# PhucNguyenAH/tacotron2_subword

Hardware: AMD Instinct MI355X
Metric: mel_frames_per_sec_train (higher is better)
Workload: dtype bf16; 1 GPU; BERT_Tacotron2 default hparams (SMA), full training iteration fwd+loss+bwd+clip+Adam, B=64/GPU, 100 phones, 60 sub-word tokens, 400 frames, 80-mel; global_batch=64, frames_per_item=400, parallelism=dp1, torch_ops=loss reductions, cat/transpose copies, persistent_chains=True, recurrent_steps_bf16=True

## Files before the change

### include/t2amd.h

```cpp
#ifndef T2AMD_H
#define T2AMD_H
#include <stddef.h>
#include <stdint.h>

#ifdef __cplusplus
extern "C" {
#endif

#define T2_ATTN_SMA 0
#define T2_ATTN_LSA 1
#define T2_ATTN_DCA 4
#define T2_ATTN_GMM 3
#define T2_ATTN_FWD2 2

enum {
    T2_SITE_PRENET1 = 1, T2_SITE_PRENET2 = 2, T2_SITE_PRENET1_SUB = 3, T2_SITE_PRENET2_SUB = 4,
    T2_SITE_ATT_H = 5, T2_SITE_ATT_C = 6, T2_SITE_ATT_H_SUB = 7, T2_SITE_ATT_C_SUB = 8,
    T2_SITE_DEC_H = 9, T2_SITE_DEC_C = 10, T2_SITE_NOISE = 11, T2_SITE_NOISE_SUB = 12,
    T2_SITE_ENC0 = 16,
    T2_SITE_ENCSUB0 = 20,
    T2_SITE_POSTNET0 = 24
};

const char* t2_last_error(void);
#define T2_ABI_VERSION 4
int t2_version(void);
int t2_chain_status(uint32_t* out_host );
int t2_chain_status_clear(void);
int t2_debug_report_abort(uint32_t code, void* stream);
int t2_debug_occupy(int workgroups, int milliseconds, void* stream);
int t2_chain_claimed(void);
int t2_set_precision(int mode);
int t2_get_precision(void);
int t2_gemm_counts(uint64_t* out_host , int reset);
int t2_set_gemm_split_min_mflop(int mflop);
int t2_set_split_steps(int on);
int t2_get_split_steps(void);
int t2_step_counts(uint64_t* out_host , int reset);
int t2_set_overlap(int on);
int t2_set_chain(int on);
int t2_get_chain(void);
int t2_set_chain_bwd(int on);
int t2_set_gemm_staging(int on);
int t2_set_gemm_fold(int on);
int t2_set_bn_fuse(int on);
int t2_get_bn_fuse(void);
int t2_bn_fuse_counts(uint64_t* out_host , int reset);
int t2_side_join(void* stream);

typedef struct t2_dims {
    int n_mel;
    int prenet_dim;
    int enc_dim;
    int att_rnn_dim;
    int dec_rnn_dim;
    int att_dim;
    int loc_filters;
    int loc_kernel;
    int attention_kind;
    float p_att_dropout, p_dec_dropout, p_prenet_dropout;
    int n_streams;
    float score_mask_value, score_mask_value_sub;
    int score_mask_given;
} t2_dims;

typedef struct t2_attention_weights {
    const float* wq;
    const float* wm;
    const float* v;
    const float* loc_conv;
    const float* loc_dense;
    const float* mlp_b1;
    const float* mlp_w2;
    const float* mlp_b2;
    const float* dca_T;
    const float* dca_bT;
    const float* dca_P;
} t2_attention_weights;
typedef struct t2_lstm_weights { const float *w_ih, *w_hh, *b_ih, *b_hh; } t2_lstm_weights;
typedef struct t2_decoder_weights {
    const float *prenet_w1, *prenet_w2;
// ... 323 lines not shown
```

### tacotron2_subword_amd/_lib.py

```python
from __future__ import annotations

import ctypes as C
import os

import torch

_HERE = os.path.dirname(os.path.abspath(__file__))
LIB_PATH = os.environ.get("T2AMD_LIB") or os.path.join(_HERE, "libt2amd.so")

ATTN_SMA, ATTN_LSA, ATTN_FWD2, ATTN_GMM, ATTN_DCA = 0, 1, 2, 3, 4

SITE = dict(PRENET1=1, PRENET2=2, PRENET1_SUB=3, PRENET2_SUB=4, ATT_H=5, ATT_C=6, ATT_H_SUB=7, ATT_C_SUB=8,
            DEC_H=9, DEC_C=10, NOISE=11, NOISE_SUB=12, ENC0=16, ENCSUB0=20, POSTNET0=24)

_fp = C.POINTER(C.c_float)
_ip = C.POINTER(C.c_int32)


class Dims(C.Structure):
    _fields_ = [("n_mel", C.c_int), ("prenet_dim", C.c_int), ("enc_dim", C.c_int), ("att_rnn_dim", C.c_int),
                ("dec_rnn_dim", C.c_int), ("att_dim", C.c_int), ("loc_filters", C.c_int), ("loc_kernel", C.c_int),
                ("attention_kind", C.c_int), ("p_att_dropout", C.c_float), ("p_dec_dropout", C.c_float),
                ("p_prenet_dropout", C.c_float), ("n_streams", C.c_int),
                ("score_mask_value", C.c_float), ("score_mask_value_sub", C.c_float), ("score_mask_given", C.c_int)]
# ... 178 lines not shown


class VocoderConvArgs(C.Structure):
    _fields_ = [("B", C.c_int), ("Cin", C.c_int), ("Cout", C.c_int), ("L", C.c_int), ("k", C.c_int), ("d", C.c_int), ("u", C.c_int),
                ("x", C.c_void_p), ("w", C.c_void_p), ("bias", C.c_void_p), ("residual", C.c_void_p),
                ("y", C.c_void_p), ("packed_ws", C.c_void_p),
                ("slope", C.c_float), ("accumulate", C.c_int), ("scale", C.c_float)]


VOCODER_TIME_TILE = 128


class StftPlanInfo(C.Structure):
    _fields_ = [("bins", C.c_int), ("overlap", C.c_int), ("frame_tile", C.c_int), ("bin_tile", C.c_int), ("out_len", C.c_long),
                ("fwd_floats", C.c_size_t), ("inv_floats", C.c_size_t), ("wsq_floats", C.c_size_t), ("packed_bytes", C.c_size_t)]


class StftAnalysisArgs(C.Structure):
    _fields_ = [("B", C.c_int), ("N", C.c_int), ("hop", C.c_int), ("n", C.c_long), ("x", C.c_void_p), ("packed", C.c_void_p),
                ("re", C.c_void_p), ("im", C.c_void_p), ("mag", C.c_void_p), ("phase", C.c_void_p)]


class StftSynthesisArgs(C.Structure):
    _fields_ = [("B", C.c_int), ("N", C.c_int), ("hop", C.c_int), ("nf", C.c_int), ("mode", C.c_int), ("windowed", C.c_int),
                ("a", C.c_void_p), ("b", C.c_void_p), ("bias", C.c_void_p), ("strength", C.c_float),
                ("packed", C.c_void_p), ("y", C.c_void_p)]


STFT_FRAME_TILE = 32
STFT_POLAR, STFT_DENOISE = 0, 1

ABI_VERSION = 4

EXPORTS = ["t2_last_error", "t2_version", "t2_chain_status", "t2_chain_status_clear", "t2_debug_report_abort", "t2_debug_occupy", "t2_chain_claimed", "t2_set_precision", "t2_get_precision", "t2_gemm_counts", "t2_set_gemm_split_min_mflop", "t2_set_split_steps", "t2_get_split_steps", "t2_step_counts", "t2_set_overlap", "t2_set_chain", "t2_get_chain", "t2_set_chain_bwd", "t2_set_gemm_staging", "t2_set_gemm_fold", "t2_set_bn_fuse", "t2_get_bn_fuse", "t2_bn_fuse_counts", "t2_side_join", "t2_decoder_layout_query", "t2_decoder_forward", "t2_decoder_infer",
           "t2_decoder_bwd_layout_query", "t2_decoder_backward", "t2_prof_enable", "t2_prof_collect", "t2_adam_chunks", "t2_adam_step", "t2_adam_norm",
           "t2_conv_bn_forward", "t2_conv_bn_backward", "t2_embedding_forward", "t2_embedding_backward",
           "t2_lstm_seq_forward", "t2_lstm_seq_backward", "t2_lstm_seq_chain_ws_floats", "t2_gemm_ex", "t2_prof_gemm", "t2_gemm_plan", "t2_conv_handoff_plan", "t2_colsum", "t2_mask_btc",
           "t2_finalize_bct", "t2_mask_bt", "t2_gemm", "t2_rng_keep_mask", "t2_rng_normal",
           "t2_softdtw_plan", "t2_softdtw_dist", "t2_softdtw_forward", "t2_softdtw_backward", "t2_softdtw_dist_backward",
           "t2_hifigan_plan", "t2_hifigan_pack", "t2_hifigan_forward", "t2_vocoder_packed_floats", "t2_vocoder_conv1d", "t2_vocoder_conv_transpose1d",
           "t2_stft_plan", "t2_stft_pack", "t2_stft_analysis", "t2_stft_synthesis"]

_lib = None


def lib() -> C.CDLL:
    global _lib
    if _lib is None:
        if not os.path.exists(LIB_PATH):
            raise RuntimeError(f"{LIB_PATH} is missing: the HIP extension must be built (see __graft_entry__.build); "
                               "there is no CPU fallback for the product path")
        L = C.CDLL(LIB_PATH)
        L.t2_last_error.restype = C.c_char_p
        if L.t2_version() != ABI_VERSION:
            raise RuntimeError(f"{LIB_PATH} speaks ABI version {L.t2_version()}, this binding {ABI_VERSION}: rebuild the library "
                               "(the argument structs differ in size between versions)")
        L.t2_chain_status.argtypes = [C.POINTER(C.c_uint32)]
        L.t2_debug_report_abort.argtypes = [C.c_uint32, C.c_void_p]
        L.t2_debug_occupy.argtypes = [C.c_int, C.c_int, C.c_void_p]
        L.t2_gemm.argtypes = [C.c_void_p, C.c_void_p, C.c_void_p, C.c_int, C.c_int, C.c_int, C.c_long, C.c_long, C.c_long,
                              C.c_long, C.c_long, C.c_void_p, C.c_int, C.c_float, C.c_float, C.c_void_p, C.c_size_t,
                              C.c_int, C.c_void_p]
        L.t2_rng_keep_mask.argtypes = [C.c_uint64, C.c_uint32, C.c_uint32, C.c_float, C.c_void_p, C.c_void_p]
        L.t2_rng_normal.argtypes = [C.c_uint64, C.c_uint32, C.c_uint32, C.c_void_p, C.c_void_p]
        L.t2_decoder_layout_query.argtypes = [C.POINTER(Dims), C.c_int, C.c_int, C.c_int, C.c_int, C.POINTER(DecoderLayout)]
        L.t2_decoder_forward.argtypes = [C.POINTER(Dims), C.POINTER(DecoderWeights), C.POINTER(DecoderFwdArgs), C.c_void_p]
        L.t2_decoder_infer.argtypes = [C.POINTER(Dims), C.POINTER(DecoderWeights), C.POINTER(DecoderInferArgs), C.c_void_p]
        L.t2_decoder_bwd_layout_query.argtypes = [C.POINTER(Dims), C.c_int, C.c_int, C.c_int, C.c_int, C.POINTER(DecoderBwdLayout)]
        L.t2_decoder_backward.argtypes = [C.POINTER(Dims), C.POINTER(DecoderWeights), C.POINTER(DecoderGrads),
                                          C.POINTER(DecoderBwdArgs), C.c_void_p]
        L.t2_conv_bn_forward.argtypes = [C.POINTER(ConvBnArgs), C.c_void_p]
        L.t2_conv_bn_backward.argtypes = [C.POINTER(ConvBnBwdArgs), C.c_void_p]
        L.t2_embedding_forward.argtypes = [C.c_void_p, C.c_void_p, C.c_void_p, C.c_int, C.c_int, C.c_void_p]
        L.t2_embedding_backward.argtypes = [C.c_void_p, C.c_void_p, C.c_void_p, C.c_int, C.c_int, C.c_int, C.c_void_p]
        L.t2_lstm_seq_forward.argtypes = [C.POINTER(LstmSeqArgs), C.c_void_p]
        L.t2_lstm_seq_backward.argtypes = [C.POINTER(LstmSeqBwdArgs), C.c_void_p]
        L.t2_lstm_seq_chain_ws_floats.argtypes, L.t2_lstm_seq_chain_ws_floats.restype = [C.c_int, C.c_int, C.c_int, C.c_int], C.c_size_t
        L.t2_gemm_ex.argtypes = [C.POINTER(GemmArgs), C.c_void_p]
        L.t2_prof_gemm.argtypes = [C.POINTER(GemmArgs), C.c_int, C.POINTER(C.c_float), C.POINTER(C.c_float), C.c_void_p]
        L.t2_gemm_plan.argtypes = [C.POINTER(GemmArgs), C.POINTER(GemmPlanOpts), C.POINTER(GemmPlanInfo)]
        L.t2_conv_handoff_plan.argtypes = [C.POINTER(GemmArgs), C.POINTER(GemmPlanOpts), C.POINTER(C.c_int), C.POINTER(GemmPlanInfo)]
        L.t2_colsum.argtypes = [C.c_void_p, C.c_long, C.c_int, C.c_int, C.c_void_p, C.c_void_p, C.c_void_p]
        L.t2_mask_btc.argtypes = [C.c_void_p, C.c_int, C.c_int, C.c_int, C.c_void_p, C.c_float, C.c_void_p]
        L.t2_prof_enable.argtypes = [C.c_int]
        L.t2_gemm_counts.argtypes = [C.POINTER(C.c_uint64), C.c_int]
        L.t2_set_split_steps.argtypes = [C.c_int]
        L.t2_step_counts.argtypes = [C.POINTER(C.c_uint64), C.c_int]
        L.t2_bn_fuse_counts.argtypes = [C.POINTER(C.c_uint64), C.c_int]
        L.t2_set_gemm_split_min_mflop.argtypes = [C.c_int]
        L.t2_prof_collect.argtypes = [C.c_int, C.POINTER(C.c_double), C.POINTER(C.c_int)]
        L.t2_finalize_bct.argtypes = [C.c_void_p, C.c_void_p, C.c_int, C.c_int, C.c_int, C.c_void_p, C.c_float, C.c_void_p]
        L.t2_mask_bt.argtypes = [C.c_void_p, C.c_int, C.c_int, C.c_void_p, C.c_float, C.c_void_p]
        L.t2_softdtw_plan.argtypes = [C.c_int, C.c_int, C.c_int, C.c_float, C.c_int, C.POINTER(SoftDtwPlanInfo)]
        L.t2_softdtw_dist.argtypes = [C.POINTER(SoftDtwDistArgs), C.c_void_p]
        L.t2_softdtw_forward.argtypes = [C.POINTER(SoftDtwFwdArgs), C.c_void_p]
        L.t2_softdtw_backward.argtypes = [C.POINTER(SoftDtwBwdArgs), C.c_void_p]
        L.t2_softdtw_dist_backward.argtypes = [C.POINTER(SoftDtwDistBwdArgs), C.c_void_p]
        L.t2_hifigan_plan.argtypes = [C.POINTER(HifiganConfig), C.c_int, C.c_int, C.POINTER(HifiganPlanInfo)]
        L.t2_hifigan_pack.argtypes = [C.POINTER(HifiganConfig), C.POINTER(C.c_void_p), C.POINTER(C.c_void_p), C.c_int, C.c_void_p, C.c_void_p]
        L.t2_hifigan_forward.argtypes = [C.POINTER(HifiganConfig), C.POINTER(HifiganFwdArgs), C.c_void_p]
        L.t2_vocoder_packed_floats.argtypes, L.t2_vocoder_packed_floats.restype = [C.c_int, C.c_int, C.c_int, C.c_int], C.c_size_t
        L.t2_vocoder_conv1d.argtypes = [C.POINTER(VocoderConvArgs), C.c_void_p]
        L.t2_vocoder_conv_transpose1d.argtypes = [C.POINTER(VocoderConvArgs), C.c_void_p]
        L.t2_stft_plan.argtypes = [C.c_int, C.c_int, C.c_int, C.POINTER(StftPlanInfo)]
        L.t2_stft_pack.argtypes = [C.c_int, C.c_int, C.c_void_p, C.c_void_p, C.c_void_p, C.c_void_p, C.c_void_p]
        L.t2_stft_analysis.argtypes = [C.POINTER(StftAnalysisArgs), C.c_void_p]
        L.t2_stft_synthesis.argtypes = [C.POINTER(StftSynthesisArgs), C.c_void_p]
        _lib = L
    return _lib


def check(rc: int) -> None:
    if rc != 0:
        raise RuntimeError(f"t2amd call failed ({rc}): {lib().t2_last_error().decode()}")


def ptr(t: torch.Tensor | None) -> int | None:
    if t is None:
        return None
    if not t.is_cuda:
        raise RuntimeError("t2amd: tensors must live on the GPU (no CPU fallback in the product path)")
# ... 204 lines not shown
    check(lib().t2_step_counts(out, int(bool(reset))))
    return tuple(int(v) for v in out)


def gemm_plan(args: GemmArgs, **opts) -> dict:
    o, info = GemmPlanOpts(**opts), GemmPlanInfo()
    check(lib().t2_gemm_plan(C.byref(args), C.byref(o), C.byref(info)))
    return dict(kernel=info.kernel, name=info.name.decode(), split=bool(info.split), splitk=info.splitk, kchunks=info.kchunks,
                a_src=info.a_src, b_src=info.b_src, stage_bytes_a=info.stage_bytes_a, stage_bytes_b=info.stage_bytes_b)


def conv_handoff_plan(args: GemmArgs, **opts) -> dict:
    o, info, taken = GemmPlanOpts(**opts), GemmPlanInfo(), C.c_int(0)
    check(lib().t2_conv_handoff_plan(C.byref(args), C.byref(o), C.byref(taken), C.byref(info)))
    return dict(taken=bool(taken.value), kernel=info.kernel, name=info.name.decode(), split=bool(info.split), splitk=info.splitk,
                kchunks=info.kchunks, a_src=info.a_src, b_src=info.b_src, stage_bytes_a=info.stage_bytes_a, stage_bytes_b=info.stage_bytes_b)


def set_gemm_fold(on: bool) -> None:
    check(lib().t2_set_gemm_fold(1 if on else 0))


def set_bn_fuse(on: bool) -> None:
    check(lib().t2_set_bn_fuse(1 if on else 0))


def get_bn_fuse() -> bool:
    return bool(lib().t2_get_bn_fuse())


def bn_fuse_counts(reset: bool = False):
    out = (C.c_uint64 * 3)()
    check(lib().t2_bn_fuse_counts(out, int(bool(reset))))
    return tuple(int(v) for v in out)


def set_gemm_split_min_mflop(mflop: int = -1) -> None:
    check(lib().t2_set_gemm_split_min_mflop(int(mflop)))


def softdtw_plan(B: int, N: int, M: int, gamma: float = 1.0, need_grad: bool = False) -> SoftDtwPlanInfo:
    info = SoftDtwPlanInfo()
    check(lib().t2_softdtw_plan(B, N, M, gamma, int(bool(need_grad)), C.byref(info)))
    return info


def hifigan_config(h) -> HifiganConfig:
    g = (lambda k: h[k]) if isinstance(h, dict) else (lambda k: getattr(h, k))
    rates, ukernels = list(g("upsample_rates")), list(g("upsample_kernel_sizes"))
    rkernels, rdil = list(g("resblock_kernel_sizes")), [list(d) for d in g("resblock_dilation_sizes")]
    kind = str(g("resblock"))
    if not kind.lstrip("-").isdigit():
        raise RuntimeError(f"hifigan: resblock \"{kind}\" is not \"1\" or \"2\"")
    if len(rates) != len(ukernels) or len(rkernels) != len(rdil):
        raise RuntimeError("hifigan: upsample_rates / upsample_kernel_sizes and resblock_kernel_sizes / resblock_dilation_sizes must pair up")
    if len(rates) > 6 or len(rkernels) > 6:
        raise RuntimeError(f"hifigan: {len(rates)} upsampling stages / {len(rkernels)} resblock kernels, at most 6 each")
    nd = len(rdil[0]) if rdil else 0
    if any(len(d) != nd for d in rdil) or nd > 3:
        raise RuntimeError(f"hifigan: resblock_dilation_sizes={rdil} must hold equally many (at most 3) dilations per kernel")
    c = HifiganConfig()
    c.resblock, c.n_mel, c.upsample_initial_channel = int(kind), 80, int(g("upsample_initial_channel"))
    c.num_upsamples, c.num_kernels, c.num_dilations = len(rates), len(rkernels), nd
    for i, (u, k) in enumerate(zip(rates, ukernels)):
        c.upsample_rates[i], c.upsample_kernel_sizes[i] = int(u), int(k)
    for j, (k, ds) in enumerate(zip(rkernels, rdil)):
# ... 17 lines not shown
```

### tacotron2_subword_amd/csrc/c_api.hip

```cpp
#include <fcntl.h>
#include <stdarg.h>
#include <stdio.h>
#include <sys/file.h>
#include <unistd.h>
#include <stdlib.h>
#include <string.h>

#include "../../include/t2amd.h"
#include "kernels.h"
#include "driver.h"

static thread_local char g_err[512] = "";

void t2_set_error(const char* fmt, ...) {
    va_list ap;
    va_start(ap, fmt);
    vsnprintf(g_err, sizeof(g_err), fmt, ap);
    va_end(ap);
}

#include <algorithm>
#include <mutex>
#include <vector>

using namespace t2;

namespace t2 {
struct Prof {
    bool on = false;
    std::vector<hipEvent_t> ev;
    std::vector<int> kind;
    size_t used = 0;
};
static Prof g_prof;

ProfScope::ProfScope(int kind, hipStream_t st) : s(st), on(g_prof.on && g_prof.used + 2 <= g_prof.ev.size()) {
    if (on) { g_prof.kind[g_prof.used / 2] = kind; (void)hipEventRecord(g_prof.ev[g_prof.used], s); }
}
ProfScope::~ProfScope() {
    if (on) { (void)hipEventRecord(g_prof.ev[g_prof.used + 1], s); g_prof.used += 2; }
}

static Side g_side[16];
int g_overlap = 1;
int g_chain = getenv("T2_CHAIN") ? atoi(getenv("T2_CHAIN")) : 1;
int g_chain_bwd = getenv("T2_CHAIN_BWD") ? atoi(getenv("T2_CHAIN_BWD")) : 1;
uint64_t g_step_counts[6] = {0, 0, 0, 0, 0, 0};
int counted(int rc, int base, int family) { if (rc == 0) ++g_step_counts[base + family]; return rc; }
int g_split_steps = getenv("T2_SPLIT_STEPS") ? atoi(getenv("T2_SPLIT_STEPS")) != 0 : 0;
int side_get(Side** out) {
    int dev = 0;
    T2_CHECK_HIP(hipGetDevice(&dev));
    Side& sd = g_side[dev & 15];
    if (!sd.s) {
        int least = 0, greatest = 0;
        T2_CHECK_HIP(hipDeviceGetStreamPriorityRange(&least, &greatest));
        T2_CHECK_HIP(hipStreamCreateWithPriority(&sd.s, hipStreamNonBlocking, least));
    }
    *out = &sd;
    return 0;
}
static int side_event(Side& sd, size_t i, hipEvent_t* out) {
    while (sd.ev.size() <= i) {
        hipEvent_t e;
        T2_CHECK_HIP(hipEventCreateWithFlags(&e, hipEventDisableTiming));
        sd.ev.push_back(e);
    }
    *out = sd.ev[i];
    return 0;
}
int stream_edge(Side& sd, size_t i, hipStream_t from, hipStream_t to) {
    hipEvent_t e;
    T2_TRY_RC(side_event(sd, i, &e));
    T2_CHECK_HIP(hipEventRecord(e, from));
    T2_CHECK_HIP(hipStreamWaitEvent(to, e, 0));
    return 0;
}

static StopPoll g_poll[16];
int stop_poll_get(StopPoll** out) {
    int dev = 0;
// ... 102 lines not shown
    T2_LAUNCH_CHECK();
    return 0;
}
int t2_set_precision(int mode) {
    T2_REQUIRE(mode >= 0 && mode <= 2, "t2_set_precision: mode must be 0 (fp32), 1 (bf16 operands) or 2 (split-bf16 large GEMMs), not %d", mode);
    set_precision(mode);
    return 0;
}
int t2_get_precision(void) { return get_precision(); }
int t2_set_gemm_split_min_mflop(int mflop) { set_gemm_split_min_mflop(mflop); return 0; }
int t2_gemm_counts(uint64_t* out_host, int reset) {
    T2_REQUIRE(out_host, "null argument");
    gemm_counts(out_host, reset);
    return 0;
}
int t2_set_split_steps(int on) { g_split_steps = on != 0; return 0; }
int t2_get_split_steps(void) { return g_split_steps; }
int t2_step_counts(uint64_t* out_host, int reset) {
    T2_REQUIRE(out_host, "null argument");
    for (int i = 0; i < 6; ++i) { out_host[i] = g_step_counts[i]; if (reset) g_step_counts[i] = 0; }
    return 0;
}
int t2_set_overlap(int on) { g_overlap = on != 0; return 0; }
int t2_set_chain(int on) { g_chain = on != 0; return 0; }
int t2_get_chain(void) { return g_chain; }
int t2_set_chain_bwd(int on) { g_chain_bwd = on != 0; return 0; }
int t2_set_gemm_staging(int on) { set_gemm_staging(on); return 0; }
int t2_set_gemm_fold(int on) { set_gemm_fold(on); return 0; }
int t2_set_bn_fuse(int on) { set_bn_fuse(on); return 0; }
int t2_get_bn_fuse(void) { return get_bn_fuse(); }
int t2_bn_fuse_counts(uint64_t* out_host, int reset) {
    T2_REQUIRE(out_host, "null argument");
    bn_fuse_counts(out_host, reset);
    return 0;
}
int t2_side_join(void* stream) {
    Side* side = nullptr;
    T2_TRY(side_get(&side));
    hipEvent_t e;
    T2_TRY(side_event(*side, 0, &e));
    T2_CHECK_HIP(hipEventRecord(e, side->s));
    T2_CHECK_HIP(hipStreamWaitEvent((hipStream_t)stream, e, 0));
    return 0;
}

int t2_conv_bn_forward(const t2_conv_bn_args* a, void* stream) {
    T2_REQUIRE(a, "null argument");
    const size_t nw = (size_t)a->Cout * a->Cin * a->K;
    T2_REQUIRE(a->ws_floats >= nw + 128 * (size_t)a->Cout, "t2_conv_bn_forward: workspace too small");
    ConvBnFwd f{};
    f.x = a->x; f.B = a->B; f.T = a->T; f.Cin = a->Cin; f.Cout = a->Cout; f.K = a->K;
    f.w = a->w; f.bias = a->bias; f.gamma = a->gamma; f.beta = a->beta; f.run_mean = a->run_mean; f.run_var = a->run_var;
    f.training = a->training; f.eps = a->eps; f.act = a->act; f.drop_p = a->drop_p; f.seed = a->seed; f.site = a->site;
    f.residual = a->residual; f.z = a->z; f.mean = a->mean; f.invstd = a->invstd; f.var = a->var; f.y = a->y;
    f.wperm = a->ws; f.scratch = a->ws + align4(nw);
    const size_t used = align4(nw) + 128 * (size_t)a->Cout;
    if (a->ws_floats > used) { f.gemm_ws = a->ws + used; f.gemm_ws_bytes = (a->ws_floats - used) * sizeof(float); }
    f.handoff = a->handoff; f.x16 = static_cast<const __bf16*>(a->x16); f.y16 = static_cast<__bf16*>(a->y16);
    return conv_bn_fwd(f, (hipStream_t)stream);
}

int t2_conv_bn_backward(const t2_conv_bn_bwd_args* a, void* stream) {
    T2_REQUIRE(a, "null argument");
    const size_t nw = align4((size_t)a->Cout * a->Cin * a->K), ndz = align4((size_t)a->B * a->T * a->Cout), nsc = 128 * (size_t)a->Cout;
    T2_REQUIRE(a->ws_floats >= nw + ndz + nsc, "t2_conv_bn_backward: workspace too small");
    ConvBnBwd f{};
// ... 358 lines not shown
```

### tacotron2_subword_amd/csrc/decoder.hip

```cpp
#include <stdlib.h>
#include <string.h>

#include <algorithm>
#include <mutex>
#include <unordered_map>
#include <vector>

#include "../../include/t2amd.h"
#include "kernels.h"
#include "driver.h"

using namespace t2;

__global__ __launch_bounds__(256) void poison_if_aborted_kernel(const unsigned* __restrict__ status, int nwords, float* __restrict__ a, size_t na,
                                                                float* __restrict__ b, size_t nb) {
    unsigned any = 0;
    for (int i = 0; i < nwords; ++i) any |= status[i];
    if (!any) return;
    const float qnan = __builtin_nanf("");
    for (size_t i = (size_t)blockIdx.x * 256 + threadIdx.x; i < na; i += (size_t)gridDim.x * 256) a[i] = qnan;
    for (size_t i = (size_t)blockIdx.x * 256 + threadIdx.x; i < nb; i += (size_t)gridDim.x * 256) b[i] = qnan;
}

namespace {
// ... 499 lines not shown
    L->dp2 = take(BT * z.P); L->dp2s = take(BT * z.P); L->dp1 = take(BT * z.P);
    L->dmel_t = take(BT * z.M); L->dgate_t = take(BT);
    L->dg16a = take((size_t)2 * z.B * 4 * z.Ha / 2 + 4); L->dg16d = take((size_t)z.B * 4 * z.Hd / 2 + 4);
    L->colsum_ws = take((size_t)64 * 4 * (z.Ha > z.Hd ? z.Ha : z.Hd));
    L->gemm_ws_floats = (size_t)192 << 20;
    if (get_precision() == 2) {
        const size_t h4 = (size_t)4 * std::max(z.Ha, z.Hd), need = 6 * BT * (h4 + z.WD) + ((size_t)256 << 20);
        L->gemm_ws_floats = std::max(L->gemm_ws_floats, align4(need / sizeof(float)));
    }
    L->gemm_ws = take(L->gemm_ws_floats);
    L->chain_floats = chain_bwd_ws_floats(lsa ? CHAIN_LSA : CHAIN_SMA, z.NS, z.B, z.Ha, z.E, z.A, d.loc_filters, d.loc_kernel, z.Hd);
    L->chain = take(L->chain_floats);
    L->total_floats = off;
}

struct BwdStreamRef {
    const t2_lstm_grads* lg; const t2_attention_grads* ag; float *prenet_w1, *prenet_w2;
    const float* d_align; float* d_memory;
    size_t dg, dctx, dq, dv, dpm, carry, carryc, dlconv, dldense, dc, dp2;
};
void bwd_stream_refs(const t2_decoder_grads& g, const t2_decoder_bwd_args& a, const t2_decoder_bwd_layout& BL, BwdStreamRef* st) {
    for (int s = 0; s < 2; ++s) {
        BwdStreamRef& b = st[s];
        b.lg = s ? &g.att_sub : &g.att; b.ag = s ? &g.attn_sub : &g.attn;
        b.prenet_w1 = s ? g.prenet_sub_w1 : g.prenet_w1; b.prenet_w2 = s ? g.prenet_sub_w2 : g.prenet_w2;
        b.d_align = s ? a.d_align_sub : a.d_align; b.d_memory = s ? a.d_memory_sub : a.d_memory;
        b.dg = s ? BL.dgas : BL.dga; b.dctx = s ? BL.dctxs : BL.dctx; b.dq = s ? BL.dqs : BL.dq; b.dv = s ? BL.dvs : BL.dv;
        b.dpm = s ? BL.dpms : BL.dpm; b.carry = s ? BL.carrys : BL.carry; b.carryc = s ? BL.carrycs : BL.carryc;
        b.dlconv = s ? BL.dlconvs : BL.dlconv; b.dldense = s ? BL.dldenses : BL.dldense;
        b.dc = s ? BL.dcas : BL.dca; b.dp2 = s ? BL.dp2s : BL.dp2;
    }
}

struct Bwd {
    const t2_dims& d; const t2_decoder_weights& w; const t2_decoder_grads& g; const t2_decoder_bwd_args& a;
    Sizes z; t2_decoder_layout L; t2_decoder_bwd_layout BL; hipStream_t s;
    const float* W(size_t off) const { return a.ws + off; }
    float* S(size_t off) const { return a.bws + off; }
    long R(int t) const { return (long)t * z.B; }
    bool use16 = false;
    bool split = false;
    hipStream_t sd = nullptr;
    const __bf16* W16(size_t off) const { return reinterpret_cast<const __bf16*>(a.ws + off); }
    __bf16* S16(size_t off) const { return reinterpret_cast<__bf16*>(a.bws + off); }
    float* gemm_ws() const { return a.bws + BL.gemm_ws; }
    size_t gemm_ws_bytes() const { return BL.gemm_ws_floats * sizeof(float); }
    StreamRef st[2]{}; BwdStreamRef bst[2]{};
    ChainBwdDesc cab{}, cbb{}; bool chain_a = false, chain_b = false;
    Side* side = nullptr; bool overlap = false; size_t ne = 0;
};

GemmDesc matmul_nn(const float* X, long ldx, const float* W, long ldw, float* Y, long ldy, int M, int N, int K) {
    return product(X, ldx, 1, W, 1, ldw, Y, ldy, M, N, K);
}
GemmDesc matmul_tn(const Bwd& c, const float* G, long ldg, const float* X, long ldx, float* Y, long ldy, int M, int N, int K) {
    GemmDesc g = product(G, 1, ldg, X, 1, ldx, Y, ldy, M, N, K);
    g.ws = c.gemm_ws(); g.ws_bytes = c.gemm_ws_bytes();
    return g;
}

struct Dg16 {
    bool on; __bf16* p; long H4; float* rest; size_t rest_bytes;
    GemmDesc operand(GemmDesc m, long row0, int kmajor) const {
        if (on) { m.A16 = p + row0 * H4; m.lda16 = H4; m.a16_kmajor = kmajor; m.ws = rest; m.ws_bytes = rest_bytes; }
        return m;
    }
    GemmDesc wgrad(GemmDesc m, long row0) const { return operand(m, row0, 1); }
    GemmDesc igrad(GemmDesc m, long row0) const { return operand(m, row0, 0); }
};
size_t dg16_bytes(const Sizes& z, int H4) { return ((size_t)H4 * z.B * z.T * sizeof(__bf16) + 255) & ~(size_t)255; }
Dg16 dg16_carve(const Bwd& c, bool on, size_t off, int H4) {
    unsigned char* const at = reinterpret_cast<unsigned char*>(c.gemm_ws()) + off;
    const size_t bytes = dg16_bytes(c.z, H4);
    return Dg16{on, reinterpret_cast<__bf16*>(at), H4, reinterpret_cast<float*>(at + bytes), c.gemm_ws_bytes() - off - bytes};
}

int dec_bwd_step(const Bwd& c, int t) {
    const Sizes& z = c.z;
    const int ks = lstm_bwd_ksplit(4 * z.Hd);
    LstmBwdPointDesc p{};
    p.nstreams = 1; p.B = z.B; p.H = z.Hd; p.seed = c.a.seed; p.first = t == z.T - 1;
    p.drop_p = c.a.training ? c.d.p_dec_dropout : 0.f;
    LstmBwdStream& st = p.st[0];
    st.dh1 = c.S(c.BL.ddout) + c.R(t) * z.WO; st.lddh1 = z.WO;
    st.part = c.S(c.BL.partd); st.nparts = ks; st.part_stride = (long)z.B * z.Hd; st.ldpart = z.Hd; st.part_col = 0;
    st.gates = c.W(c.L.gd) + c.R(t) * 4 * z.Hd; st.ldgates = 4 * z.Hd;
    st.c_new = c.W(c.L.cnd) + c.R(t) * z.Hd; st.ldc_new = z.Hd;
    if (t > 0) { st.c_prev = c.W(c.L.cd) + c.R(t - 1) * z.Hd; st.ldc_prev = z.Hd; }
    st.dc_state = c.S(c.BL.dcd);
    st.dg = c.S(c.BL.dgd) + c.R(t) * 4 * z.Hd; st.lddg = 4 * z.Hd;
    st.site_h = T2_SITE_DEC_H; st.site_c = T2_SITE_DEC_C;
    st.idx_base = (uint32_t)(c.R(t) * z.Hd); st.idx_bstride = (uint32_t)z.Hd;
    if (c.use16) st.dg16 = c.S16(c.BL.dg16d);
    hipStream_t sd = c.sd ? c.sd : c.s;
    { ProfScope ps(PK_LSTM_DEC_BWD_PW, sd); T2_TRY(lstm_bwd_pointwise(p, sd)); }
    if (t == 0) return 0;
    LstmBwdGemmDesc g{};
    g.nstreams = 1; g.B = z.B; g.H4 = 4 * z.Hd; g.KS = ks; g.NC = z.Hd;
    g.st[0].dg = st.dg; g.st[0].lddg = st.lddg;
    g.st[0].seg[0] = LstmBwdSeg{c.w.dec.w_hh, (long)z.Hd, z.Hd}; g.st[0].nseg = 1;
    g.st[0].part = c.S(c.BL.partd);
    if (c.use16) { g.st[0].dg16 = c.S16(c.BL.dg16d); g.st[0].wt16 = c.W16(c.L.wt16d); }
// ... 314 lines not shown
    unsigned char* const ws8 = reinterpret_cast<unsigned char*>(c.gemm_ws());
    const size_t wt_bytes = ((size_t)4 * z.Hd * z.WD * sizeof(__bf16) + 255) & ~(size_t)255;
    const bool pre16 = get_precision() == 1 && (4 * z.Hd) % 64 == 0 && z.WD % 64 == 0 && c.gemm_ws_bytes() > 2 * wt_bytes;
    if (pre16) T2_TRY(stage_bf16(c.w.dec.w_ih, false, z.WD, reinterpret_cast<__bf16*>(ws8), z.WD, 4 * z.Hd, sb));
    const size_t dg16_off = pre16 ? wt_bytes : 0;
    const bool share = get_precision() == 1 && BT % 64 == 0 && z.B % 8 == 0 && (4 * z.Hd) % 128 == 0 && z.T > 1 &&
                       c.gemm_ws_bytes() >= dg16_off + dg16_bytes(z, 4 * z.Hd) + ((size_t)z.WD * BT * sizeof(__bf16) + 256);
    const Dg16 dg = dg16_carve(c, share, dg16_off, 4 * z.Hd);
    bool chunk_cast = share && pre16;
    for (size_t ci = 1; ci < bounds.size(); ++ci) if (((bounds[ci] - bounds[ci - 1]) * z.B) % 64 != 0) chunk_cast = false;
    c.chain_b = c.chain_a && chain_b_bwd_desc(c, &c.cbb);
    for (size_t ci = bounds.size() - 1; ci > 0; --ci) {
        const int t0 = bounds[ci - 1], t1 = bounds[ci];
        if (c.chain_b) {
            c.cbb.t0 = t0; c.cbb.t1 = t1;
            ProfScope ps(PK_CHAIN_B_BWD, sb);
            T2_TRY(chain_bwd(c.cbb, c.S(BL.chain), BL.chain_floats, sb));
        } else {
            for (int t = t1 - 1; t >= t0; --t) T2_TRY(dec_bwd_step(c, t));
        }
        GemmDesc dd = matmul_nn(DGd + c.R(t0) * 4 * z.Hd, 4 * z.Hd, c.w.dec.w_ih, z.WD, c.S(BL.ddin) + c.R(t0) * z.WD, z.WD,
                                (t1 - t0) * z.B, z.WD, 4 * z.Hd);
        dd.ws = c.gemm_ws(); dd.ws_bytes = c.gemm_ws_bytes();
        if (pre16) {
            dd.B16 = reinterpret_cast<const __bf16*>(ws8); dd.ldb16 = 4 * z.Hd;
            dd.ws = reinterpret_cast<float*>(ws8 + wt_bytes); dd.ws_bytes -= wt_bytes;
        }
        if (chunk_cast) {
            T2_TRY(stage_bf16(DGd + c.R(t0) * 4 * z.Hd, true, 4 * z.Hd, dg.p + c.R(t0) * 4 * z.Hd, (t1 - t0) * z.B, 4 * z.Hd, sb));
            dd = dg.igrad(dd, c.R(t0));
        }
        T2_TRY(gemm(dd, sb));
        if (c.overlap) T2_TRY(stream_edge(*c.side, c.ne++, sb, c.s));
        if (t0 == 0) T2_TRY(bwd_dec_lstm_wgrads(c, dg, chunk_cast, sb));
        if (c.chain_a) {
            c.cab.t0 = t0; c.cab.t1 = t1;
            ProfScope ps(PK_CHAIN_A_BWD, c.s);
            T2_TRY(chain_bwd(c.cab, c.S(BL.chain), BL.chain_floats, c.s));
        } else {
            for (int t = t1 - 1; t >= t0; --t) T2_TRY(att_bwd_step(c, t));
        }
    }
    return 0;
}

int bwd_stream_tail(const Bwd& c, int s, hipStream_t ts) {
    const Sizes& z = c.z; const t2_decoder_layout& L = c.L;
    const StreamRef& r = c.st[s]; const BwdStreamRef& b = c.bst[s];
    const t2_lstm_grads& lg = *b.lg; const t2_attention_grads& ag = *b.ag;
    const int BT = z.B * z.T, hoff = r.hoff, coff = r.coff;
    float* cws = c.S(c.BL.colsum_ws);
    const float* DG = c.S(b.dg);
    const float* DIN = c.W(L.din);
    const float* P1 = c.W(r.p1); const float* P2 = c.W(r.p2);
    float* dP2 = c.S(b.dp2); float* dP1 = c.S(c.BL.dp1);
    const long ldw = z.P + z.E;
    const bool share = get_precision() == 1 && BT % 64 == 0 && z.B % 8 == 0 && (4 * z.Ha) % 128 == 0 && z.T > 1 &&
                       c.gemm_ws_bytes() >= 2 * dg16_bytes(z, 4 * z.Ha);
    const Dg16 dg = dg16_carve(c, share, 0, 4 * z.Ha);
    if (share) T2_TRY(stage_bf16(DG, true, 4 * z.Ha, dg.p, BT, 4 * z.Ha, ts));
    const __bf16* DIN16 = share && c.use16 ? c.W16(L.din16) : nullptr;
    auto dw_gemm = [&](const float* G, long row0, const float* X, const __bf16* X16, long ldx, float* Y, long ldy, int N, int K) -> int {
        GemmDesc m = dg.wgrad(matmul_tn(c, G, 4 * z.Ha, X, ldx, Y, ldy, 4 * z.Ha, N, K), row0);
        if (X16) { m.B16 = X16; m.ldb16 = ldx; m.b16_kmajor = 1; }
        return gemm(m, ts);
    };
    T2_TRY(dw_gemm(DG, 0, P2, nullptr, z.P, lg.w_ih, ldw, z.P, BT));
// ... 27 lines not shown
    T2_TRY(gemm(matmul_tn(c, DQ, 2 * z.A, DIN + hoff, z.WD, ag.wq, z.Ha, z.A, z.Ha, BT), ts));
    const bool dcak = c.d.attention_kind == T2_ATTN_DCA;
    const bool gmm = c.d.attention_kind == T2_ATTN_GMM || dcak;
    if (dcak) {
        T2_REQUIRE(ag.mlp_b1 && ag.mlp_w2 && ag.loc_conv && ag.loc_dense && ag.dca_T && ag.dca_bT && ag.v, "t2_decoder_backward: DCA gradient buffers missing");
        T2_TRY(colsum(DQ, 2 * z.A, BT, z.A, ag.mlp_b1, nullptr, cws, ts));
        const size_t na = dca_acc_floats(z.A);
        float* full = c.gemm_ws();
        T2_REQUIRE(na * sizeof(float) <= c.gemm_ws_bytes(), "t2_decoder_backward: scratch too small");
        T2_TRY(batch_sum(c.S(b.dldense), z.B, (int)na, full, ts));
        auto cp = [&](float* dst, size_t off, size_t n) { return hipMemcpyAsync(dst, full + off, n * sizeof(float), hipMemcpyDeviceToDevice, ts); };
        size_t off = 0;
        T2_CHECK_HIP(cp(ag.v, off, z.A)); off += z.A;
        T2_CHECK_HIP(cp(ag.dca_bT, off, z.A)); off += z.A;
        T2_CHECK_HIP(cp(ag.loc_dense, off, (size_t)z.A * kDcaC)); off += (size_t)z.A * kDcaC;
        T2_CHECK_HIP(cp(ag.dca_T, off, (size_t)z.A * kDcaC)); off += (size_t)z.A * kDcaC;
        T2_CHECK_HIP(cp(ag.loc_conv, off, kDcaC * kDcaK)); off += kDcaC * kDcaK;
        T2_CHECK_HIP(cp(ag.mlp_w2, off, (size_t)kDcaC * kDcaK * z.A));
    } else if (gmm) {
        T2_REQUIRE(ag.mlp_b1 && ag.mlp_w2 && ag.mlp_b2, "t2_decoder_backward: GMM needs mlp_b1 / mlp_w2 / mlp_b2 gradient buffers");
        T2_TRY(colsum(DQ, 2 * z.A, BT, z.A, ag.mlp_b1, nullptr, cws, ts));
        T2_TRY(batch_sum(c.S(b.dldense), z.B, 3 * kGmmK * z.A, ag.mlp_w2, ts));
        float* b2tmp = cws;
        T2_TRY(batch_sum(c.S(b.dlconv), z.B, 16, b2tmp, ts));
        T2_CHECK_HIP(hipMemcpyAsync(ag.mlp_b2, b2tmp, 3 * kGmmK * sizeof(float), hipMemcpyDeviceToDevice, ts));
    } else {
        T2_TRY(batch_sum(c.S(b.dv), nsp * z.B, z.A, ag.v, ts));
    }
    if (c.d.attention_kind == T2_ATTN_LSA) {
        T2_REQUIRE(ag.loc_conv && ag.loc_dense, "t2_decoder_backward: LSA needs loc_conv / loc_dense gradient buffers");
        T2_TRY(batch_sum(c.S(b.dlconv), (lsa_chain ? 2 : 1) * z.B, c.d.loc_filters * 2 * c.d.loc_kernel, ag.loc_conv, ts));
        T2_TRY(batch_sum(c.S(b.dldense), (lsa_chain ? 2 : 1) * z.B, z.A * c.d.loc_filters, ag.loc_dense, ts));
    }
    if (!gmm) {
        const float* DPM = c.S(b.dpm);
        T2_TRY(gemm(matmul_tn(c, DPM, z.A, r.memory, z.E, ag.wm, z.E, z.A, z.E, z.B * r.Tin), ts));
        T2_TRY(gemm(matmul_nn(DPM, z.A, r.aw->wm, z.E, b.d_memory, z.E, z.B * r.Tin, z.E, z.A), c.s));
    }
    GemmDesc dm = gemm_desc();
    dm.A = r.align; dm.sam = 1; dm.sak = r.Tin; dm.bsA = (long)z.T * r.Tin;
    dm.B = c.S(b.dctx); dm.sbk = (long)z.B * z.E; dm.sbn = 1; dm.bsB = z.E;
    dm.C = b.d_memory; dm.ldc = z.E; dm.bsC = (long)r.Tin * z.E;
    dm.M = r.Tin; dm.N = z.E; dm.K = z.T; dm.batch = z.B; dm.beta = gmm ? 0.f : 1.f;
    return gemm(dm, c.s);
}

}

extern "C" {

int t2_decoder_layout_query(const t2_dims* dims_in, int B, int T, int Tin, int Tsub, t2_decoder_layout* out) {
    T2_REQUIRE(dims_in && out, "null argument");
    t2_dims d; int max_pos = 0;
    T2_TRY(entry_dims(*dims_in, &d, &max_pos));
    T2_REQUIRE(B >= 1 && B <= 256 && T >= 1 && Tin >= 1 && Tsub >= 1, "bad shape B=%d T=%d Tin=%d Tsub=%d", B, T, Tin, Tsub);
    layout_of(d, sizes_of(d, B, T, Tin, Tsub), out);
    return 0;
}

int t2_decoder_forward(const t2_dims* dims_in, const t2_decoder_weights* w, const t2_decoder_fwd_args* a, void* stream) {
    T2_REQUIRE(dims_in && w && a, "null argument");
    t2_dims d; int max_pos = 0;
    T2_TRY(entry_dims(*dims_in, &d, &max_pos));
    T2_REQUIRE(a->B >= 1 && a->B <= 256 && a->T >= 1, "bad shape B=%d T=%d", a->B, a->T);
    T2_REQUIRE((long)a->B * a->T * 4 * d.att_rnn_dim < (1l << 32), "B*T too large for 32-bit RNG indices");
    Dec c{d, *w, sizes_of(d, a->B, a->T, a->Tin, a->Tsub), a->ws, a->training != 0, a->prenet_dropout != 0, true, a->seed, (hipStream_t)stream, max_pos};
    layout_of(d, c.z, &c.L);
    stream_refs(d, *w, c.z, c.L, a->memory, a->memory_sub, a->mem_lengths, a->sub_lengths, a->align, a->align_sub, c.st);
    const Sizes& z = c.z;
    T2_REQUIRE(a->phase >= 0 && a->phase <= 2, "t2_decoder_forward: phase must be 0, 1 or 2");
    c.use16 = use_bf16_steps(z);
    c.split = use_split_steps(z);
    c.w16_bytes = ((size_t)4 * z.Hd * z.WD * sizeof(__bf16) + 255) & ~(size_t)255;
    c.pre16 = c.use16 && (4 * z.Hd) % 64 == 0 && z.WD % 64 == 0 && c.L.gemm_ws_floats * sizeof(float) > c.w16_bytes;
    if (a->phase != 2) {
        T2_TRY(fwd_prologue(c, a->mels));
        if (a->phase == 1) return 0;
    }
    T2_TRY(processed_memory(c));
    T2_TRY(fwd_chains(c));
    return fwd_outputs(c, a->mel_out, a->gate_out);
}

int t2_decoder_bwd_layout_query(const t2_dims* dims_in, int B, int T, int Tin, int Tsub, t2_decoder_bwd_layout* out) {
    T2_REQUIRE(dims_in && out, "null argument");
    t2_dims d; int max_pos = 0;
    T2_TRY(entry_dims(*dims_in, &d, &max_pos));
    T2_REQUIRE(B >= 1 && B <= 256 && T >= 1 && Tin >= 1 && Tsub >= 1, "bad shape B=%d T=%d Tin=%d Tsub=%d", B, T, Tin, Tsub);
    bwd_layout_of(d, sizes_of(d, B, T, Tin, Tsub), out);
    return 0;
}

int t2_decoder_backward(const t2_dims* dims_in, const t2_decoder_weights* w, const t2_decoder_grads* g,
                        const t2_decoder_bwd_args* a, void* stream) {
    T2_REQUIRE(dims_in && w && g && a, "null argument");
    t2_dims d; int max_pos = 0;
    T2_TRY(entry_dims(*dims_in, &d, &max_pos));
    Bwd c{d, *w, *g, *a, sizes_of(d, a->B, a->T, a->Tin, a->Tsub), {}, {}, (hipStream_t)stream};
    layout_of(d, c.z, &c.L);
    bwd_layout_of(d, c.z, &c.BL);
    stream_refs(d, *w, c.z, c.L, a->memory, a->memory_sub, nullptr, nullptr, const_cast<float*>(a->align), const_cast<float*>(a->align_sub), c.st);
    bwd_stream_refs(*g, *a, c.BL, c.bst);
    c.use16 = use_bf16_steps(c.z);
    c.split = use_split_steps(c.z);
    T2_TRY(bwd_projections(c));
    T2_TRY(bwd_chains(c));
    const bool defer = c.overlap && a->defer_weight_grads != 0;
    hipStream_t ts = c.s;
    if (defer) {
        T2_TRY(stream_edge(*c.side, c.ne++, c.s, c.side->s));
        ts = c.side->s;
    } else if (c.overlap) {
        T2_TRY(stream_edge(*c.side, c.ne++, c.side->s, c.s));
    }
    for (int s = 0; s < c.z.NS; ++s) T2_TRY(bwd_stream_tail(c, s, ts));
    return 0;
}

int t2_decoder_infer(const t2_dims* dims_in, const t2_decoder_weights* w, const t2_decoder_infer_args* a, void* stream) {
    T2_REQUIRE(dims_in && w && a && a->steps_run_host, "null argument");
    t2_dims d; int max_pos = 0;
    T2_TRY(entry_dims(*dims_in, &d, &max_pos));
    T2_REQUIRE(a->B >= 1 && a->B <= 256 && a->max_steps >= 1, "bad shape B=%d max_steps=%d", a->B, a->max_steps);
    Dec c{d, *w, sizes_of(d, a->B, a->max_steps, a->Tin, a->Tsub), a->ws, false, a->prenet_dropout != 0, false, a->seed, (hipStream_t)stream, max_pos};
    layout_of(d, c.z, &c.L);
    stream_refs(d, *w, c.z, c.L, a->memory, a->memory_sub, a->mem_lengths, a->sub_lengths, a->align, a->align_sub, c.st);
    const Sizes& z = c.z; const t2_decoder_layout& L = c.L;
    const int T = z.T;
    int poll = a->poll_every > 0 ? a->poll_every : 16;

    hipLaunchKernelGGL(init_stop_kernel, dim3((z.B + 63) / 64), dim3(64), 0, c.s, a->stop_index, a->done_count, z.B);
    T2_LAUNCH_CHECK();
    T2_TRY(processed_memory(c));
    for (int s = 0; s < z.NS; ++s)
        T2_TRY(permute_rows(c.st[s].prenet_w1, c.P(L.w1t) + (size_t)s * z.M * z.P, z.P, z.M, 1, c.s));
    c.I = infer_shadows(z, L.w16a);
    c.use16 = get_precision() == 1 && z.B <= 128 && c.I.Ka % 256 == 0 && c.I.Kd % 256 == 0;
    if (c.use16) {
        const long ldi = z.P + z.E;
        for (int s = 0; s < z.NS; ++s) {
            const t2_lstm_weights& lw = *c.st[s].lw;
            __bf16* f = c.P16(c.I.wa[s]);
            T2_TRY(cast_part(lw.w_hh, z.Ha, f, 0, c.I.Ka, 4 * z.Ha, z.Ha, false, false, c.s));
            T2_TRY(cast_part(lw.w_ih + z.P, ldi, f + z.Ha, 0, c.I.Ka, 4 * z.Ha, z.E, false, false, c.s));
            T2_TRY(cast_part(lw.w_ih, ldi, f + z.Ha + z.E, 0, c.I.Ka, 4 * z.Ha, z.P, false, false, c.s));
        }
        T2_TRY(cast_part(w->dec.w_ih, z.WD, c.P16(c.I.wd), 0, c.I.Kd, 4 * z.Hd, z.WD, false, false, c.s));
        T2_TRY(cast_part(w->dec.w_hh, z.Hd, c.P16(c.I.wd) + z.WD, 0, c.I.Kd, 4 * z.Hd, z.Hd, false, false, c.s));
// ... 66 lines not shown
```

### tacotron2_subword_amd/csrc/driver.h

```cpp
#pragma once
#include <hip/hip_runtime.h>
#include <stdint.h>

#include <vector>

#define T2_TRY(expr)                \
    do {                            \
        int rc_ = (expr);           \
        if (rc_ != 0) return rc_;   \
    } while (0)

namespace t2 {

enum ProfKind { PK_LSTM_ATT_FWD = 0, PK_ATTN_FWD, PK_LSTM_DEC_FWD, PK_ATTN_BWD, PK_LSTM_ATT_BWD_PW, PK_LSTM_ATT_BWD_GEMM,
                PK_LSTM_DEC_BWD_PW, PK_LSTM_DEC_BWD_GEMM, PK_CHAIN_A_FWD, PK_CHAIN_B_FWD, PK_CHAIN_B_BWD, PK_CHAIN_A_BWD, PK_CHAIN_DEC, PK_COUNT };
struct ProfScope {
    hipStream_t s; bool on;
    ProfScope(int kind, hipStream_t st);
    ~ProfScope();
};

struct Side { hipStream_t s = nullptr; std::vector<hipEvent_t> ev; };
int side_get(Side** out);
int stream_edge(Side& sd, size_t i, hipStream_t from, hipStream_t to);

struct StopPoll { hipEvent_t ev[4] = {}; int32_t* host = nullptr; };
int stop_poll_get(StopPoll** out);

extern int g_overlap, g_chain, g_chain_bwd, g_split_steps;

extern uint64_t g_step_counts[6];
int counted(int rc, int base, int family);

}
```

### tacotron2_subword_amd/model.py

```python
from math import sqrt

import torch
from torch import nn

from . import _lib as L
from . import blocks
from . import ops
from .attention import (DynamicConvolutionAttention, ForwardAttentionV2, GMMAttention, LocationSensitiveAttention,
                        StepwiseMonotonicAttention)
from .layers import ConvNorm, LinearNorm
from .utils import get_mask_from_lengths, to_gpu


class Prenet(nn.Module):

    def __init__(self, in_dim, sizes):
        super().__init__()
        ins = [in_dim] + sizes[:-1]
        self.layers = nn.ModuleList([LinearNorm(i, o, bias=False) for i, o in zip(ins, sizes)])


class Postnet(nn.Module):

    def __init__(self, hparams):
# ... 122 lines not shown
        self.single = bool(single)
        ns = 1 if single else 2
        self.n_mel_channels, self.n_frames_per_step = hp.n_mel_channels, hp.n_frames_per_step
        self.encoder_embedding_dim, self.attention_rnn_dim = hp.encoder_embedding_dim, hp.attention_rnn_dim
        self.decoder_rnn_dim, self.prenet_dim = hp.decoder_rnn_dim, hp.prenet_dim
        self.max_decoder_steps, self.gate_threshold = hp.max_decoder_steps, hp.gate_threshold
        self.p_attention_dropout, self.p_decoder_dropout = hp.p_attention_dropout, hp.p_decoder_dropout
        E, Ha, Hd, Pn = hp.encoder_embedding_dim, hp.attention_rnn_dim, hp.decoder_rnn_dim, hp.prenet_dim
        M = hp.n_mel_channels * hp.n_frames_per_step
        self.prenet = Prenet(M, [Pn, Pn])
        if not single:
            self.prenet_bert = Prenet(M, [Pn, Pn])
        self.attention_rnn = nn.LSTMCell(Pn + E, Ha)
        if not single:
            self.attention_rnn_bert = nn.LSTMCell(Pn + E, Ha)
        att_cls = {"StepwiseMonotonicAttention": StepwiseMonotonicAttention, "ForwardAttentionV2": ForwardAttentionV2,
                   "GMMAttention": GMMAttention, "DynamicConvolutionAttention": DynamicConvolutionAttention,
                   "LSA": LocationSensitiveAttention, "LocationSensitiveAttention": LocationSensitiveAttention}.get(hp.attention)
        if att_cls is None:
            att_cls = LocationSensitiveAttention
        print({"SMA": "Use SMA", "LSA": "Use LSA", "FWD2": "Use ForwardAttention", "GMM": "Use GMMA",
               "DCA": "Use DCA"}[att_cls.kind])
        args = (Ha, E, hp.attention_dim, hp.attention_location_n_filters, hp.attention_location_kernel_size)
        self.attention_layer = att_cls(*args)
        if not single:
            self.attention_layer_bert = att_cls(*args)
        self.decoder_rnn = nn.LSTMCell(ns * (Ha + E), Hd, 1)
        if not single:
            self.decoder_rnn_bert = nn.LSTMCell(Ha + E, Hd, 1)
        self.linear_projection = LinearNorm(Hd + ns * E, M)
        self.gate_layer = LinearNorm(Hd + ns * E, 1, bias=True, w_init_gain="sigmoid")
        self._dims = L.dims_from_hparams(hp, ns)
        self.prenet_dropout = True
        self.defer_weight_grads = False
        self.base_seed, self._calls = int(getattr(hp, "seed", 1234)), 0

    @property
    def dims(self):
        d = self._dims
        d.score_mask_value = float(self.attention_layer.score_mask_value)
        d.score_mask_given = 1
        if not self.single:
            d.score_mask_value_sub = float(self.attention_layer_bert.score_mask_value)
        return d

    def _param_keys(self):
        return L.decoder_param_keys(self.dims.attention_kind, self.single)

    def _params(self):
        sd = dict(self.named_parameters())
        return [sd[k] for k in self._param_keys()]

    def _next_seed(self):
        return _next_seed(self)

    def _weights(self):
        P = {"decoder." + k: v.detach() for k, v in self.named_parameters()}
        P.update({"decoder." + k: v for k, v in self.named_buffers()})
        return P, L.decoder_weights(P, self.dims.attention_kind, single=self.single)

    def prologue(self, decoder_inputs, B, Tin, Tsub):
        seed = self._next_seed()
        mels = decoder_inputs.contiguous()
        _, W = self._weights()
        dp = ops.DecoderPass(self.dims, B, mels.shape[2], Tin, Tsub, mels.device)
        cur = torch.cuda.current_stream()
        if getattr(self, "_pro_stream", None) is None:
# ... 181 lines not shown
```

Baseline: 1.035 million mel-frames/s.

## Defer decoder LSTM weight grads and attention tail to side stream in backward

Turns on deferred weight-gradient computation by default and, when chained backward is active, postpones the decoder LSTM weight-gradient GEMMs from inside the recurrent chain to a side stream after the chains finish. The d_memory input-gradient GEMMs are split out of the stream tail so they stay on the main stream, while the weight-gradient tails run concurrently on the side stream. The aim is to shorten the critical path of the serial recurrent backward by moving weight-gradient work off it and overlapping it. It adds a debug counter, relies on the side stream being joined correctly, and keeps the staged bf16 gradient buffer alive longer.

```diff
diff --git a/include/t2amd.h b/include/t2amd.h
--- a/include/t2amd.h
+++ b/include/t2amd.h
@@ -47,6 +47,7 @@
 int t2_get_bn_fuse(void);
 int t2_bn_fuse_counts(uint64_t* out_host , int reset);
 int t2_side_join(void* stream);
+int t2_defer_counts(uint64_t* out_host , int reset);
 
 typedef struct t2_dims {
     int n_mel;
diff --git a/tacotron2_subword_amd/_lib.py b/tacotron2_subword_amd/_lib.py
--- a/tacotron2_subword_amd/_lib.py
+++ b/tacotron2_subword_amd/_lib.py
@@ -234,7 +234,7 @@
 
 ABI_VERSION = 4
 
-EXPORTS = ["t2_last_error", "t2_version", "t2_chain_status", "t2_chain_status_clear", "t2_debug_report_abort", "t2_debug_occupy", "t2_chain_claimed", "t2_set_precision", "t2_get_precision", "t2_gemm_counts", "t2_set_gemm_split_min_mflop", "t2_set_split_steps", "t2_get_split_steps", "t2_step_counts", "t2_set_overlap", "t2_set_chain", "t2_get_chain", "t2_set_chain_bwd", "t2_set_gemm_staging", "t2_set_gemm_fold", "t2_set_bn_fuse", "t2_get_bn_fuse", "t2_bn_fuse_counts", "t2_side_join", "t2_decoder_layout_query", "t2_decoder_forward", "t2_decoder_infer",
+EXPORTS = ["t2_last_error", "t2_version", "t2_chain_status", "t2_chain_status_clear", "t2_debug_report_abort", "t2_debug_occupy", "t2_chain_claimed", "t2_set_precision", "t2_get_precision", "t2_gemm_counts", "t2_set_gemm_split_min_mflop", "t2_set_split_steps", "t2_get_split_steps", "t2_step_counts", "t2_set_overlap", "t2_set_chain", "t2_get_chain", "t2_set_chain_bwd", "t2_set_gemm_staging", "t2_set_gemm_fold", "t2_set_bn_fuse", "t2_get_bn_fuse", "t2_bn_fuse_counts", "t2_side_join", "t2_defer_counts", "t2_decoder_layout_query", "t2_decoder_forward", "t2_decoder_infer",
            "t2_decoder_bwd_layout_query", "t2_decoder_backward", "t2_prof_enable", "t2_prof_collect", "t2_adam_chunks", "t2_adam_step", "t2_adam_norm",
            "t2_conv_bn_forward", "t2_conv_bn_backward", "t2_embedding_forward", "t2_embedding_backward",
            "t2_lstm_seq_forward", "t2_lstm_seq_backward", "t2_lstm_seq_chain_ws_floats", "t2_gemm_ex", "t2_prof_gemm", "t2_gemm_plan", "t2_conv_handoff_plan", "t2_colsum", "t2_mask_btc",
@@ -289,6 +289,7 @@
         L.t2_set_split_steps.argtypes = [C.c_int]
         L.t2_step_counts.argtypes = [C.POINTER(C.c_uint64), C.c_int]
         L.t2_bn_fuse_counts.argtypes = [C.POINTER(C.c_uint64), C.c_int]
+        L.t2_defer_counts.argtypes = [C.POINTER(C.c_uint64), C.c_int]
         L.t2_set_gemm_split_min_mflop.argtypes = [C.c_int]
         L.t2_prof_collect.argtypes = [C.c_int, C.POINTER(C.c_double), C.POINTER(C.c_int)]
         L.t2_finalize_bct.argtypes = [C.c_void_p, C.c_void_p, C.c_int, C.c_int, C.c_int, C.c_void_p, C.c_float, C.c_void_p]
@@ -559,6 +560,12 @@
 def bn_fuse_counts(reset: bool = False):
     out = (C.c_uint64 * 3)()
     check(lib().t2_bn_fuse_counts(out, int(bool(reset))))
+    return tuple(int(v) for v in out)
+
+
+def defer_counts(reset: bool = False):
+    out = (C.c_uint64 * 2)()
+    check(lib().t2_defer_counts(out, int(bool(reset))))
     return tuple(int(v) for v in out)
 
 
diff --git a/tacotron2_subword_amd/csrc/c_api.hip b/tacotron2_subword_amd/csrc/c_api.hip
--- a/tacotron2_subword_amd/csrc/c_api.hip
+++ b/tacotron2_subword_amd/csrc/c_api.hip
@@ -47,6 +47,7 @@
 int g_chain_bwd = getenv("T2_CHAIN_BWD") ? atoi(getenv("T2_CHAIN_BWD")) : 1;
 uint64_t g_step_counts[6] = {0, 0, 0, 0, 0, 0};
 int counted(int rc, int base, int family) { if (rc == 0) ++g_step_counts[base + family]; return rc; }
+uint64_t g_defer_counts[2] = {0, 0};
 int g_split_steps = getenv("T2_SPLIT_STEPS") ? atoi(getenv("T2_SPLIT_STEPS")) != 0 : 0;
 int side_get(Side** out) {
     int dev = 0;
@@ -215,6 +216,11 @@
 int t2_bn_fuse_counts(uint64_t* out_host, int reset) {
     T2_REQUIRE(out_host, "null argument");
     bn_fuse_counts(out_host, reset);
+    return 0;
+}
+int t2_defer_counts(uint64_t* out_host, int reset) {
+    T2_REQUIRE(out_host, "null argument");
+    for (int i = 0; i < 2; ++i) { out_host[i] = g_defer_counts[i]; if (reset) g_defer_counts[i] = 0; }
     return 0;
 }
 int t2_side_join(void* stream) {
diff --git a/tacotron2_subword_amd/csrc/decoder.hip b/tacotron2_subword_amd/csrc/decoder.hip
--- a/tacotron2_subword_amd/csrc/decoder.hip
+++ b/tacotron2_subword_amd/csrc/decoder.hip
@@ -555,6 +555,16 @@
     }
 }
 
+struct Dg16 {
+    bool on; __bf16* p; long H4; float* rest; size_t rest_bytes;
+    GemmDesc operand(GemmDesc m, long row0, int kmajor) const {
+        if (on) { m.A16 = p + row0 * H4; m.lda16 = H4; m.a16_kmajor = kmajor; m.ws = rest; m.ws_bytes = rest_bytes; }
+        return m;
+    }
+    GemmDesc wgrad(GemmDesc m, long row0) const { return operand(m, row0, 1); }
+    GemmDesc igrad(GemmDesc m, long row0) const { return operand(m, row0, 0); }
+};
+
 struct Bwd {
     const t2_dims& d; const t2_decoder_weights& w; const t2_decoder_grads& g; const t2_decoder_bwd_args& a;
     Sizes z; t2_decoder_layout L; t2_decoder_bwd_layout BL; hipStream_t s;
@@ -571,6 +581,7 @@
     StreamRef st[2]{}; BwdStreamRef bst[2]{};
     ChainBwdDesc cab{}, cbb{}; bool chain_a = false, chain_b = false;
     Side* side = nullptr; bool overlap = false; size_t ne = 0;
+    bool defer = false; Dg16 dgd16{}; bool dgd16_staged = false;
 };
 
 GemmDesc matmul_nn(const float* X, long ldx, const float* W, long ldw, float* Y, long ldy, int M, int N, int K) {
@@ -582,15 +593,6 @@
     return g;
 }
 
-struct Dg16 {
-    bool on; __bf16* p; long H4; float* rest; size_t rest_bytes;
-    GemmDesc operand(GemmDesc m, long row0, int kmajor) const {
-        if (on) { m.A16 = p + row0 * H4; m.lda16 = H4; m.a16_kmajor = kmajor; m.ws = rest; m.ws_bytes = rest_bytes; }
-        return m;
-    }
-    GemmDesc wgrad(GemmDesc m, long row0) const { return operand(m, row0, 1); }
-    GemmDesc igrad(GemmDesc m, long row0) const { return operand(m, row0, 0); }
-};
 size_t dg16_bytes(const Sizes& z, int H4) { return ((size_t)H4 * z.B * z.T * sizeof(__bf16) + 255) & ~(size_t)255; }
 Dg16 dg16_carve(const Bwd& c, bool on, size_t off, int H4) {
     unsigned char* const at = reinterpret_cast<unsigned char*>(c.gemm_ws()) + off;
@@ -971,7 +973,8 @@
         }
         T2_TRY(gemm(dd, sb));
         if (c.overlap) T2_TRY(stream_edge(*c.side, c.ne++, sb, c.s));
-        if (t0 == 0) T2_TRY(bwd_dec_lstm_wgrads(c, dg, chunk_cast, sb));
+        if (t0 == 0 && c.chain_a && c.defer) { c.dgd16 = dg; c.dgd16_staged = chunk_cast; }
+        else if (t0 == 0) T2_TRY(bwd_dec_lstm_wgrads(c, dg, chunk_cast, sb));
         if (c.chain_a) {
             c.cab.t0 = t0; c.cab.t1 = t1;
             ProfScope ps(PK_CHAIN_A_BWD, c.s);
@@ -1065,11 +1068,15 @@
         T2_TRY(batch_sum(c.S(b.dlconv), (lsa_chain ? 2 : 1) * z.B, c.d.loc_filters * 2 * c.d.loc_kernel, ag.loc_conv, ts));
         T2_TRY(batch_sum(c.S(b.dldense), (lsa_chain ? 2 : 1) * z.B, z.A * c.d.loc_filters, ag.loc_dense, ts));
     }
-    if (!gmm) {
-        const float* DPM = c.S(b.dpm);
-        T2_TRY(gemm(matmul_tn(c, DPM, z.A, r.memory, z.E, ag.wm, z.E, z.A, z.E, z.B * r.Tin), ts));
-        T2_TRY(gemm(matmul_nn(DPM, z.A, r.aw->wm, z.E, b.d_memory, z.E, z.B * r.Tin, z.E, z.A), c.s));
-    }
+    if (!gmm) T2_TRY(gemm(matmul_tn(c, c.S(b.dpm), z.A, r.memory, z.E, ag.wm, z.E, z.A, z.E, z.B * r.Tin), ts));
+    return 0;
+}
+
+int bwd_stream_dmemory(const Bwd& c, int s) {
+    const Sizes& z = c.z;
+    const StreamRef& r = c.st[s]; const BwdStreamRef& b = c.bst[s];
+    const bool gmm = c.d.attention_kind == T2_ATTN_GMM || c.d.attention_kind == T2_ATTN_DCA;
+    if (!gmm) T2_TRY(gemm(matmul_nn(c.S(b.dpm), z.A, r.aw->wm, z.E, b.d_memory, z.E, z.B * r.Tin, z.E, z.A), c.s));
     GemmDesc dm = gemm_desc();
     dm.A = r.align; dm.sam = 1; dm.sak = r.Tin; dm.bsA = (long)z.T * r.Tin;
     dm.B = c.S(b.dctx); dm.sbk = (long)z.B * z.E; dm.sbn = 1; dm.bsB = z.E;
@@ -1136,17 +1143,21 @@
     bwd_stream_refs(*g, *a, c.BL, c.bst);
     c.use16 = use_bf16_steps(c.z);
     c.split = use_split_steps(c.z);
+    c.defer = g_overlap && c.z.T >= 32 && a->defer_weight_grads != 0;
     T2_TRY(bwd_projections(c));
     T2_TRY(bwd_chains(c));
-    const bool defer = c.overlap && a->defer_weight_grads != 0;
     hipStream_t ts = c.s;
-    if (defer) {
+    if (c.defer) {
+        if (!c.side) T2_TRY(side_get(&c.side));
         T2_TRY(stream_edge(*c.side, c.ne++, c.s, c.side->s));
         ts = c.side->s;
+        if (c.chain_a) T2_TRY(bwd_dec_lstm_wgrads(c, c.dgd16, c.dgd16_staged, ts));
     } else if (c.overlap) {
         T2_TRY(stream_edge(*c.side, c.ne++, c.side->s, c.s));
     }
+    for (int s = 0; s < c.z.NS; ++s) T2_TRY(bwd_stream_dmemory(c, s));
     for (int s = 0; s < c.z.NS; ++s) T2_TRY(bwd_stream_tail(c, s, ts));
+    ++g_defer_counts[c.defer ? 0 : 1];
     return 0;
 }
 
diff --git a/tacotron2_subword_amd/csrc/driver.h b/tacotron2_subword_amd/csrc/driver.h
--- a/tacotron2_subword_amd/csrc/driver.h
+++ b/tacotron2_subword_amd/csrc/driver.h
@@ -32,4 +32,6 @@
 extern uint64_t g_step_counts[6];
 int counted(int rc, int base, int family);
 
+extern uint64_t g_defer_counts[2];
+
 }
diff --git a/tacotron2_subword_amd/model.py b/tacotron2_subword_amd/model.py
--- a/tacotron2_subword_amd/model.py
+++ b/tacotron2_subword_amd/model.py
@@ -178,7 +178,7 @@
         self.gate_layer = LinearNorm(Hd + ns * E, 1, bias=True, w_init_gain="sigmoid")
         self._dims = L.dims_from_hparams(hp, ns)
         self.prenet_dropout = True
-        self.defer_weight_grads = False
+        self.defer_weight_grads = True
         self.base_seed, self._calls = int(getattr(hp, "seed", 1234)), 0
 
     @property
```

Result: faster. 1.059 million mel-frames/s, median of 6 (+2.4%).
